# impromptuRong/hd_yolo

Hardware: AMD Instinct MI355X
Metric: tiles/sec (640x640) fwd+bwd (higher is better)
Workload: dtype bf16; 1 GPU; metayolo yolov5s 8-class nuclei, 640x640 RGB tiles, batch 64/GPU, train step = fwd + DetLoss + bwd + all-reduce + SGD(nesterov); global_batch=64, parallelism=dp1, world_size=1, backend=none, hw_queues=4

## Files before the change

### hd_yolo_amd/csrc/api.hip

```cpp
#include <stdarg.h>
#include <stdio.h>
#include <stdlib.h>
#include <string.h>

#include <atomic>

#include "common.h"
#include "hdyolo_internal.h"
#include "hdyolo.h"

int hdy_pack_weight_launch(const hdy_pack_desc& d, hipStream_t st);
int hdy_pack_batch_launch(const hdy_pack_desc* table, int n, int total_blocks, hipStream_t st);

static thread_local char g_err[512] = "";

void hdy_set_error(const char* fmt, ...) {
    va_list ap;
    va_start(ap, fmt);
    vsnprintf(g_err, sizeof(g_err), fmt, ap);
    va_end(ap);
}

namespace {
struct OptDef { const char* name; int def; bool flag; };
const OptDef g_opt_def[HDY_OPT_COUNT] = {
    {"HDY_NO_CLASS_WALK", 0, true}, {"HDY_NO_CONV3X3", 0, true}, {"HDY_C3_GRID", 0, false}, {"HDY_NO_CONV3X3S2", 0, false},
    {"HDY_NO_DGRAD_S2", 0, false}, {"HDY_TILE_INTERLEAVE", 1, false}, {"HDY_NO_BIG_TILES", 0, true}, {"HDY_NO_STEM_KERNEL", 0, true},
    {"HDY_WGRAD_BLOCKS", 512, false}, {"HDY_NO_STEM_WGRAD", 0, true}, {"HDY_NO_WGRAD3X3", 0, true}, 
    {"HDY_LOSS_GRID", 2048, false}, {"HDY_NO_DEEP", 0, true}, {"HDY_NO_WGRAD_DEEP", 0, true}, {"HDY_DEEP_BN", 0, false}, {"HDY_DEEP_DEBUG", 0, false}, {"HDY_DEEP_ALL", 1, false}, {"HDY_DEEP_MIN_TILES", 160, false}, {"HDY_DEEP_WALK", 2, false}, {"HDY_NO_BN_REDUCE4", 0, true},
    {"HDY_WGRAD_TILE", 0, false}, {"HDY_SPPF_NO_KEYS", 0, true}, {"HDY_WGRAD_DEEP_KMIN", 192, false}, {"HDY_NO_CONV3X3_C128", 0, true}, {"HDY_NO_F1X1_96", 0, true},
    {"HDY_AP_CHUNK", 0, false}, {"HDY_AP_NO_PRUNE", 0, true},
};
std::atomic<int> g_opt[HDY_OPT_COUNT];
std::once_flag g_opt_once;
void opt_init() {
    std::call_once(g_opt_once, [] {
        for (int i = 0; i < HDY_OPT_COUNT; ++i) {
            const char* v = getenv(g_opt_def[i].name);
            g_opt[i].store(v ? (g_opt_def[i].flag ? 1 : atoi(v)) : g_opt_def[i].def, std::memory_order_relaxed);
        }
    });
}
int opt_index(const char* name) {
    for (int i = 0; name && i < HDY_OPT_COUNT; ++i)
        if (!strcmp(name, g_opt_def[i].name)) return i;
    return -1;
}
thread_local char g_disp_last[64] = "";
std::mutex g_disp_mu;
char g_disp_log[32768] = "";
size_t g_disp_len = 0;
thread_local char g_disp_copy[32768] = "";
}

int hdy_opt(int id) {
    opt_init();
    return g_opt[id].load(std::memory_order_relaxed);
}

void hdy_note_dispatch(const char* what) {
    snprintf(g_disp_last, sizeof(g_disp_last), "%s", what);
    const size_t n = strlen(g_disp_last);
    std::lock_guard<std::mutex> lock(g_disp_mu);
    if (g_disp_len + n + 2 < sizeof(g_disp_log)) {
        memcpy(g_disp_log + g_disp_len, g_disp_last, n);
        g_disp_log[g_disp_len + n] = ';';
        g_disp_log[g_disp_len + n + 1] = 0;
        g_disp_len += n + 1;
    }
}

namespace {

enum { KIND_FWD = 0, KIND_DGRAD = 1, KIND_STEM = 2 };

inline int velems(int dtype) { return dtype == HDY_BF16 ? 8 : 4; }
inline int bke(int dtype) { return 8 * velems(dtype); }
inline size_t esize(int dtype) { return dtype == HDY_BF16 ? 2 : 4; }

inline size_t block_elems(int rows, int kd, int dtype) {
    const int bn = hdy_conv_bn_tile(rows);
    return (size_t)round_up(rows, bn) * round_up(kd, bke(dtype));
}

}

extern "C" {

const char* hdy_last_error(void) { return g_err; }

const char* hdy_last_dispatch(void) { return g_disp_last; }

const char* hdy_dispatch_log(void) {
    std::lock_guard<std::mutex> lock(g_disp_mu);
    memcpy(g_disp_copy, g_disp_log, g_disp_len + 1);
    return g_disp_copy;
}

void hdy_dispatch_log_reset(void) {
    std::lock_guard<std::mutex> lock(g_disp_mu);
    g_disp_log[0] = 0;
    g_disp_len = 0;
    g_disp_last[0] = 0;
}

int hdy_set_option(const char* name, int value) {
    const int i = opt_index(name);
    HDY_ARG(i >= 0, "set_option: unknown option %s", name ? name : "(null)");
    opt_init();
    return g_opt[i].exchange(value, std::memory_order_relaxed);
}

int hdy_get_option(const char* name) {
    const int i = opt_index(name);
    HDY_ARG(i >= 0, "get_option: unknown option %s", name ? name : "(null)");
    return hdy_opt(i);
}

int hdy_version(void) { return HDY_ABI_VERSION; }

int hdy_fastdiv_magic(unsigned d, unsigned* magic, int* shift) {
    HDY_ARG(d > 0 && magic && shift, "fastdiv_magic: d must be positive");
    hdy_magic(d, magic, shift);
    return HDY_OK;
}

int hdy_conv_out_dim(int in, int k, int stride, int pad) { return conv_out_dim(in, k, stride, pad); }

int hdy_conv_mtiles(long long M) { return (int)((M + 127) / 128); }

size_t hdy_conv_pack_elems(int K, int C, int R, int S, int stride, int pad, int kind, int dtype) {
    if (kind == KIND_FWD) return block_elems(K, R * S * C, dtype);
    if (kind == KIND_STEM) return block_elems(K, R * S * 4, dtype);
    if (stride == 1) return block_elems(C, R * S * K, dtype);
    size_t n = 0;
    for (int a = 0; a < 2; ++a)
        for (int b = 0; b < 2; ++b) {
            const Axis ah = class_axis(R, pad, a), aw = class_axis(S, pad, b);
            if (ah.taps && aw.taps) n += block_elems(C, ah.taps * aw.taps * K, dtype);
        }
    return n;
}

static hdy_pack_desc make_desc(const float* w_a, int K_a, const float* w_b, int K_b, void* out, int Kl, int C, int R, int S, int transpose,
                               int TH, int TW, int rbase, int rstep, int sbase, int sstep, int stem, int rows_total, int Kdp, int dtype,
                               int first_block) {
    hdy_pack_desc d = {};
    d.w_a = w_a; d.w_b = w_b; d.out = out; d.K_a = K_a; d.K_b = K_b; d.Kl = Kl; d.C = C; d.R = R; d.S = S; d.transpose = transpose;
    d.TH = TH; d.TW = TW; d.rbase = rbase; d.rstep = rstep; d.sbase = sbase; d.sstep = sstep; d.stem = stem; d.rows_total = rows_total;
    d.Kdp = Kdp; d.dtype = dtype; d.first_block = first_block;
    d.nblocks = cdiv((long long)rows_total * Kdp, 2048);
    return d;
}

int hdy_conv_pack_describe(const float* w_a, int K_a, const float* w_b, int K_b, int K, int C, int R, int S, int stride, int pad, int kind,
                           int dtype, void* out, hdy_pack_desc* descs, int first_block) {
    HDY_ARG(w_a && out && descs && K_a > 0 && K_b >= 0 && K >= K_a + K_b && C > 0 && R > 0 && S > 0, "conv_pack: bad args");
    HDY_ARG((K_b == 0) == (w_b == nullptr), "conv_pack: w_b / K_b mismatch");
    HDY_ARG(stride == 1 || stride == 2, "conv_pack: stride %d unsupported", stride);
    HDY_ARG(dtype == HDY_BF16 || dtype == HDY_F32, "conv_pack: unknown dtype %d", dtype);
    HDY_ARG(((long long)K + 256) * ((long long)R * S * ((long long)C + 256) + 64) < (1LL << 31), "conv_pack: weight too large for 32-bit packing indices");
    if (kind == KIND_FWD || kind == KIND_STEM) {
        const int stem = kind == KIND_STEM;
        HDY_ARG(!stem || (C == 3 && K_b == 0), "conv_pack: stem expects C == 3 and a single weight");
        const int kd = stem ? R * S * 4 : R * S * C;
        const int Kdp = round_up(kd, bke(dtype));
        const int rows_total = round_up(K, hdy_conv_bn_tile(K));
        descs[0] = make_desc(w_a, K_a, w_b, K_b, out, K, C, R, S, 0, R, stem ? 1 : S, 0, 1, 0, 1, stem, rows_total, Kdp, dtype, first_block);
        return 1;
    }
    HDY_ARG(kind == KIND_DGRAD, "conv_pack: unknown kind %d", kind);
    const int rows_total = round_up(C, hdy_conv_bn_tile(C));
    if (stride == 1) {
        const int Kdp = round_up(R * S * K, bke(dtype));
        descs[0] = make_desc(w_a, K_a, w_b, K_b, out, K, C, R, S, 1, R, S, R - 1, -1, S - 1, -1, 0, rows_total, Kdp, dtype, first_block);
        return 1;
    }
    size_t off = 0;
    int n = 0;
    for (int a = 0; a < 2; ++a)
        for (int b = 0; b < 2; ++b) {
            const Axis ah = class_axis(R, pad, a), aw = class_axis(S, pad, b);
            if (!ah.taps || !aw.taps) continue;
            const int Kdp = round_up(ah.taps * aw.taps * K, bke(dtype));
            descs[n] = make_desc(w_a, K_a, w_b, K_b, (char*)out + off * esize(dtype), K, C, R, S, 1, ah.taps, aw.taps, ah.rmax, -2, aw.rmax,
                                 -2, 0, rows_total, Kdp, dtype, first_block);
            first_block += descs[n].nblocks;
            off += (size_t)rows_total * Kdp;
            ++n;
        }
    return n;
}

int hdy_conv_pack(const float* w_a, int K_a, const float* w_b, int K_b, int K, int C, int R, int S, int stride, int pad, int kind,
                  int dtype, void* out, void* stream) {
    hdy_pack_desc d[4];
    const int n = hdy_conv_pack_describe(w_a, K_a, w_b, K_b, K, C, R, S, stride, pad, kind, dtype, out, d, 0);
    if (n < 0) return n;
    for (int i = 0; i < n; ++i) {
        const int rc = hdy_pack_weight_launch(d[i], (hipStream_t)stream);
        if (rc) return rc;
    }
    return HDY_OK;
}

int hdy_conv_pack_run(const hdy_pack_desc* descs_device, int ndesc, int total_blocks, void* stream) {
    HDY_ARG(descs_device && ndesc > 0 && total_blocks > 0, "conv_pack_run: bad args");
    return hdy_pack_batch_launch(descs_device, ndesc, total_blocks, (hipStream_t)stream);
}

}
```

### hd_yolo_amd/csrc/common.h

```cpp
#pragma once
#include <hip/hip_runtime.h>
#include <stdint.h>
#include <stddef.h>

#include <mutex>

#define HDY_OK 0
#define HDY_EINVAL (-1)
#define HDY_EUNSUPPORTED (-2)

enum { HDY_F32 = 0, HDY_BF16 = 1 };

void hdy_set_error(const char* fmt, ...);

enum HdyOption {
    HDY_OPT_NO_CLASS_WALK,
    HDY_OPT_NO_CONV3X3,
    HDY_OPT_C3_GRID,
    HDY_OPT_NO_CONV3X3S2,
    HDY_OPT_NO_DGRAD_S2,
    HDY_OPT_TILE_INTERLEAVE,
    HDY_OPT_NO_BIG_TILES,
    HDY_OPT_NO_STEM_KERNEL,
    HDY_OPT_WGRAD_BLOCKS,
    HDY_OPT_NO_STEM_WGRAD,
    HDY_OPT_NO_WGRAD3X3,
    HDY_OPT_LOSS_GRID,
    HDY_OPT_NO_DEEP,
    HDY_OPT_NO_WGRAD_DEEP,
    HDY_OPT_DEEP_BN,
    HDY_OPT_DEEP_DEBUG,
    HDY_OPT_DEEP_ALL,
    HDY_OPT_DEEP_MIN_TILES,
    HDY_OPT_DEEP_WALK,
    HDY_OPT_NO_BN_REDUCE4,
    HDY_OPT_WGRAD_TILE,
    HDY_OPT_SPPF_NO_KEYS,
    HDY_OPT_WGRAD_DEEP_KMIN,
    HDY_OPT_NO_CONV3X3_C128,
    HDY_OPT_NO_F1X1_96,
    HDY_OPT_AP_CHUNK,
    HDY_OPT_AP_NO_PRUNE,
    HDY_OPT_COUNT
};
int hdy_opt(int id);

void hdy_note_dispatch(const char* what);

#define HDY_ARG(cond, ...)                 \
    do {                                   \
        if (!(cond)) {                     \
            hdy_set_error(__VA_ARGS__);    \
            return HDY_EINVAL;             \
        }                                  \
    } while (0)

#define HDY_LAUNCH_CHECK(what)                                                       \
    do {                                                                             \
        hipError_t e__ = hipGetLastError();                                          \
        if (e__ != hipSuccess) {                                                     \
            hdy_set_error("%s: launch failed: %s", what, hipGetErrorString(e__));    \
            return (int)e__;                                                         \
        }                                                                            \
    } while (0)

typedef __bf16 bf16_t;
typedef int i32x4 __attribute__((ext_vector_type(4)));
typedef float f32x4 __attribute__((ext_vector_type(4)));
typedef __bf16 bf16x8 __attribute__((ext_vector_type(8)));
typedef __bf16 bf16x4 __attribute__((ext_vector_type(4)));

#if defined(__HIPCC__)
__device__ __forceinline__ float row_sum16(float v) {
#ifdef HDY_ROW_SUM_SHFL
    for (int m = 1; m < 16; m <<= 1) v += __shfl_xor(v, m);
    return v;
#endif
    v += __builtin_bit_cast(float, __builtin_amdgcn_update_dpp(0, __builtin_bit_cast(int, v), 0x128, 0xF, 0xF, true));
    v += __builtin_bit_cast(float, __builtin_amdgcn_update_dpp(0, __builtin_bit_cast(int, v), 0x124, 0xF, 0xF, true));
    v += __builtin_bit_cast(float, __builtin_amdgcn_update_dpp(0, __builtin_bit_cast(int, v), 0x122, 0xF, 0xF, true));
    v += __builtin_bit_cast(float, __builtin_amdgcn_update_dpp(0, __builtin_bit_cast(int, v), 0x121, 0xF, 0xF, true));
    return v;
}
#endif

struct PerDeviceOnce {
    std::once_flag flag[16];
    template <typename F> void run(F&& fn) {
        int dev = 0;
        (void)hipGetDevice(&dev);
        std::call_once(flag[dev & 15], fn);
    }
};

static inline int cdiv(long long a, long long b) { return (int)((a + b - 1) / b); }
static inline int round_up(int a, int b) { return (a + b - 1) / b * b; }

#ifdef __HIPCC__
union V16 {
    i32x4 i;
    f32x4 f;
    bf16x8 h;
};

__device__ __forceinline__ float silu_f(float u) { return u / (1.0f + __expf(-u)); }
__device__ __forceinline__ float sigmoid_f(float u) { return 1.0f / (1.0f + __expf(-u)); }

template <typename T> __device__ __forceinline__ float to_f32(T v);
template <> __device__ __forceinline__ float to_f32<float>(float v) { return v; }
template <> __device__ __forceinline__ float to_f32<bf16_t>(bf16_t v) { return (float)v; }
template <typename T> __device__ __forceinline__ T from_f32(float v);
template <> __device__ __forceinline__ float from_f32<float>(float v) { return v; }
template <> __device__ __forceinline__ bf16_t from_f32<bf16_t>(float v) { return (bf16_t)v; }

__device__ __forceinline__ int xcd_remap(int id, int n) {
    const int q = n >> 3, r = n & 7, x = id & 7, s = id >> 3;
    return (x < r ? x * (q + 1) : r * (q + 1) + (x - r) * q) + s;
}
__device__ __forceinline__ unsigned fdiv(unsigned n, unsigned mg, int sh) { return __umulhi(n << 1, mg) >> sh; }

__device__ __forceinline__ bool iou_gt(float ax1, float ay1, float ax2, float ay2, float aarea, float bx1, float by1, float bx2, float by2,
                                       float barea, float thr) {
    const float xx1 = ax1 > bx1 ? ax1 : bx1;
    const float yy1 = ay1 > by1 ? ay1 : by1;
    const float xx2 = ax2 < bx2 ? ax2 : bx2;
    const float yy2 = ay2 < by2 ? ay2 : by2;
    float w = __fsub_rn(xx2, xx1);
    float h = __fsub_rn(yy2, yy1);
    w = w < 0.f ? 0.f : w;
    h = h < 0.f ? 0.f : h;
    const float inter = __fmul_rn(w, h);
    const float ovr = __fdiv_rn(inter, __fsub_rn(__fadd_rn(aarea, barea), inter));
    return ovr > thr;
}

__device__ __forceinline__ unsigned desc_key(float s) {
    unsigned u = s == 0.0f ? 0u : __float_as_uint(s);
    u = (u & 0x80000000u) ? ~u : (u | 0x80000000u);
    return ~u;
}

__device__ __forceinline__ void glds16(const void* g, unsigned char* lds_wave_base) {
    __builtin_amdgcn_global_load_lds((const void __attribute__((address_space(1)))*)g,
                                     (void __attribute__((address_space(3)))*)lds_wave_base, 16, 0, 0);
}

__device__ __forceinline__ void lds_dma16(__amdgpu_buffer_rsrc_t r, unsigned voff, unsigned soff, unsigned char* lds_wave_base) {
    __builtin_amdgcn_raw_ptr_buffer_load_lds(r, (void __attribute__((address_space(3)))*)lds_wave_base, 16, (int)voff, (int)soff, 0, 0);
}

__device__ __forceinline__ void lds_dma16(__amdgpu_buffer_rsrc_t r, unsigned voff, unsigned soff, unsigned lds_byte) {
    __builtin_amdgcn_raw_ptr_buffer_load_lds(r, (void __attribute__((address_space(3)))*)(uintptr_t)lds_byte, 16, (int)voff, (int)soff, 0, 0);
}

__device__ __forceinline__ int fsw(int row) { return ((row >> 1) & 1) | (((row >> 3) & 1) << 1); }
__device__ __forceinline__ int fsw3(int row) { return (row & 6) ^ (((row >> 3) & 1) * 5); }

__device__ __forceinline__ float fast_sigmoid(float u) { return __builtin_amdgcn_rcpf(1.0f + __expf(-u)); }
__device__ __forceinline__ float dsilu_f(float u) {
    const float s = fast_sigmoid(u);
    return s * (1.0f + u * (1.0f - s));
}

template <typename T> __device__ __forceinline__ void unpack(const i32x4& v, float* f);
template <> __device__ __forceinline__ void unpack<float>(const i32x4& v, float* f) {
    V16 u; u.i = v;
#pragma unroll
    for (int i = 0; i < 4; ++i) f[i] = u.f[i];
}
template <> __device__ __forceinline__ void unpack<bf16_t>(const i32x4& v, float* f) {
    V16 u; u.i = v;
#pragma unroll
    for (int i = 0; i < 8; ++i) f[i] = (float)u.h[i];
}
template <typename T> __device__ __forceinline__ i32x4 pack(const float* f);
template <> __device__ __forceinline__ i32x4 pack<float>(const float* f) {
    V16 u;
#pragma unroll
    for (int i = 0; i < 4; ++i) u.f[i] = f[i];
    return u.i;
}
template <> __device__ __forceinline__ i32x4 pack<bf16_t>(const float* f) {
    V16 u;
#pragma unroll
    for (int i = 0; i < 8; ++i) u.h[i] = (bf16_t)f[i];
    return u.i;
}

#define VEC_OK(ptr, ld, VE) ((((uintptr_t)(ptr)) & 15) == 0 && (ld) % (VE) == 0)

#define S2_LDSR(dst, addr)                                                                             \
    do {                                                                                               \
        if constexpr (HAND) asm volatile("ds_read_b128 %0, %1" : "=v"(dst) : "v"(addr) : "memory");    \
        else dst = *(const i32x4*)(smem + ((addr) - lds0));                                            \
    } while (0)
#define S2_LGKM(n)                                                                                                       \
    do {                                                                                                                 \
        if constexpr (HAND) { asm volatile("s_waitcnt lgkmcnt(%0)" ::"n"(n) : "memory"); __builtin_amdgcn_sched_barrier(0); } \
    } while (0)
#define S2_BARRIER(lg)                                                                                                   \
    do {                                                                                                                 \
        if constexpr (HAND) { if (lg) asm volatile("s_waitcnt lgkmcnt(0)" ::: "memory"); __builtin_amdgcn_s_barrier(); asm volatile("" ::: "memory"); } \
        else __syncthreads();                                                                                            \
    } while (0)
#endif
```

### hd_yolo_amd/csrc/conv_dgrad_s2.hip

```cpp
#include <stdlib.h>

#include "common.h"
#include "hdyolo_internal.h"

__device__ uint4 g_hdy_zero16_d2[4];

namespace {

constexpr int TW = 16, PW = TW + 1;
constexpr int CB = 128, CPP = 8;

template <int NP, int NCG, int TH> struct Geo {
    static constexpr int NWP = TH / 4;
    static constexpr int NTHR = 64 * NCG * NWP;
    static constexpr int PPIX = (TH + 1) * PW;
    static constexpr int PLANE_B = PPIX * CB;
    static constexpr int PATCH_B = NP * PLANE_B;
    static constexpr int PPR = 4 / NCG;
    static constexpr int RPH = 32 / PPR;
    static constexpr int SROWS = 2 * TH * RPH;
    static constexpr int STAGE_B = SROWS * 128;
    static constexpr int SMEM_B = 2 * PATCH_B + STAGE_B;
    static constexpr int NPASS = (PPIX * CPP + NTHR - 1) / NTHR;
    static constexpr int RPP = NTHR / 8;
    static constexpr int SPASS = SROWS / RPP;
    static constexpr int HSTEP = RPP / RPH;
    static_assert(SPASS == 8 && RPP % RPH == 0 && PPIX <= 153, "geometry");
};

template <int NP, int NCG, int TH, int ABL = 0>
__global__ __launch_bounds__(64 * NCG * (TH / 4), 2) void dgrad3x3s2_kernel(const ConvArgs p) {
    using G = Geo<NP, NCG, TH>;
    constexpr int NTHR = G::NTHR, PATCH_B = G::PATCH_B, PLANE_B = G::PLANE_B, PPIX = G::PPIX, NPASS = G::NPASS, PPR = G::PPR, KD = 64 * NP;
    constexpr bool HAND = NP == 2;
    extern __shared__ __attribute__((aligned(16))) unsigned char smem[];
    unsigned char* sP = smem;
    unsigned char* sS = smem + 2 * PATCH_B;

    const unsigned lds0 = (unsigned)(uintptr_t)(const __attribute__((address_space(3))) unsigned char*)smem;
    const int tid = threadIdx.x, lane = tid & 63, wave = tid >> 6;
    const int fr = lane & 15, fq = lane >> 4;
    const int wc = wave % NCG, wp = wave / NCG;
    const int tiles_w = p.Wo / TW, tiles_h = p.Ho / TH, per_img = tiles_w * tiles_h;
    const int tiles = p.N * per_img;
    const int wg = xcd_remap(blockIdx.x, gridDim.x);

    const bf16_t* __restrict__ x = (const bf16_t*)p.x;
    const bf16_t* __restrict__ w = (const bf16_t*)p.w;
    const unsigned char* zero = (const unsigned char*)g_hdy_zero16_d2;

    V16 bw[9][2 * NP];
    {
        constexpr int cls_of[9] = {0, 1, 1, 2, 2, 3, 3, 3, 3}, tap_of[9] = {0, 0, 1, 0, 1, 0, 1, 2, 3};
#pragma unroll
        for (int i = 0; i < 9; ++i) {
            const bf16_t* base = w + p.c_w[cls_of[i]] + (size_t)(wc * 16 + fr) * (p.c_nkb[cls_of[i]] * 64) + tap_of[i] * KD;
#pragma unroll
            for (int kk = 0; kk < 2 * NP; ++kk) bw[i][kk].i = *(const i32x4*)(base + (kk * 4 + fq) * 8);
        }
    }

    auto issue_patch = [&](int t, int buf) {
        int tv = tid;
        if constexpr (HAND) asm volatile("" : "+v"(tv));
        const int lc = tv & 7, wv = tv >> 6;
        const int n = t / per_img, rem = t - n * per_img;
        const int th = rem / tiles_w, tw = rem - th * tiles_w;
        const int i0 = th * TH, j0 = tw * TW;
        const bf16_t* org = x + (((long long)n * p.Hin + i0) * p.Win + j0) * p.ldx;
        unsigned char* dst = sP + buf * PATCH_B;
#pragma unroll
        for (int pl = 0; pl < NP; ++pl)
#pragma unroll
            for (int i = 0; i < NPASS; ++i) {
                if ((wave * 64 + NTHR * i) / CPP >= PPIX) break;
                const int pix = (tv + NTHR * i) / CPP;
                if (pix >= PPIX) continue;
                const int py = (pix * 3856) >> 16, px = pix - py * PW;
                const int lcp = lc ^ (((px >> 1) & 3) << 1);
                const void* src = (i0 + py < p.Hin && j0 + px < p.Win) ? (const void*)(org + ((long long)py * p.Win + px) * p.ldx + pl * 64 + lcp * 8) : (const void*)zero;
                glds16(src, dst + pl * PLANE_B + (wv * 64 + NTHR * i) * 16);
            }
    };

    int aoff[2][2];
#pragma unroll
    for (int s = 0; s < 2; ++s)
#pragma unroll
        for (int ks = 0; ks < 2; ++ks) {
            const int px = fr + s;
            aoff[s][ks] = px * CB + (((ks * 4 + fq) ^ (((px >> 1) & 3) << 1)) << 4);
        }

    const int st_ch = tid & 7, st_rr = tid >> 3;
    const int st_key = PPR == 2 ? (st_rr & 15) : ((st_rr >> 1) & 15);
    const int st_lds = st_rr * 128 + ((st_ch ^ (st_key >> 1)) << 4);
    const int st_hr0 = st_rr / G::RPH;
    const long long st_pix = PPR == 2 ? (long long)(2 * (st_rr & 15) + (st_ch >> 2)) * p.ldy + (st_ch & 3) * 8 : (long long)(st_rr & 31) * p.ldy + st_ch * 8;

    auto compute = [&](int t, int cur) {
        f32x4 acc[4][4];
#pragma unroll
        for (int c = 0; c < 4; ++c)
#pragma unroll
            for (int a = 0; a < 4; ++a) acc[c][a] = f32x4{0.f, 0.f, 0.f, 0.f};
#pragma unroll
        for (int pl = 0; pl < NP; ++pl) {
            const unsigned pb = lds0 + cur * PATCH_B + pl * PLANE_B + wp * 4 * PW * CB;
            V16 f[2][2];
            S2_LDSR(f[0][0].i, pb + aoff[0][0]);
            S2_LDSR(f[0][1].i, pb + aoff[1][0]);
#pragma unroll
            for (int g = 0; g < 10; ++g) {
                const int q = g >> 1, ks = pl * 2 + (g & 1);
                if (g + 1 < 10) {
                    S2_LDSR(f[(g + 1) & 1][0].i, pb + ((g + 1) >> 1) * PW * CB + aoff[0][(g + 1) & 1]);
                    S2_LDSR(f[(g + 1) & 1][1].i, pb + ((g + 1) >> 1) * PW * CB + aoff[1][(g + 1) & 1]);
                    S2_LGKM(2);
                } else {
                    S2_LGKM(0);
                }
                const bf16x8 f0 = f[g & 1][0].h, f1 = f[g & 1][1].h;
                if (ABL & 4) continue;
                if (q < 4) {
                    acc[0][q] = __builtin_amdgcn_mfma_f32_16x16x32_bf16(bw[0][ks].h, f0, acc[0][q], 0, 0, 0);
                    acc[1][q] = __builtin_amdgcn_mfma_f32_16x16x32_bf16(bw[1][ks].h, f0, acc[1][q], 0, 0, 0);
                    acc[2][q] = __builtin_amdgcn_mfma_f32_16x16x32_bf16(bw[3][ks].h, f0, acc[2][q], 0, 0, 0);
                    acc[3][q] = __builtin_amdgcn_mfma_f32_16x16x32_bf16(bw[5][ks].h, f0, acc[3][q], 0, 0, 0);
                    acc[1][q] = __builtin_amdgcn_mfma_f32_16x16x32_bf16(bw[2][ks].h, f1, acc[1][q], 0, 0, 0);
                    acc[3][q] = __builtin_amdgcn_mfma_f32_16x16x32_bf16(bw[6][ks].h, f1, acc[3][q], 0, 0, 0);
                }
                if (q >= 1) {
                    acc[2][q - 1] = __builtin_amdgcn_mfma_f32_16x16x32_bf16(bw[4][ks].h, f0, acc[2][q - 1], 0, 0, 0);
                    acc[3][q - 1] = __builtin_amdgcn_mfma_f32_16x16x32_bf16(bw[7][ks].h, f0, acc[3][q - 1], 0, 0, 0);
                    acc[3][q - 1] = __builtin_amdgcn_mfma_f32_16x16x32_bf16(bw[8][ks].h, f1, acc[3][q - 1], 0, 0, 0);
                }
            }
        }
#pragma unroll
        for (int c = 0; c < 4; ++c)
#pragma unroll
            for (int a = 0; a < 4; ++a) {
                const int ca = c >> 1, cb = c & 1;
                const int hr = 2 * (wp * 4 + a) + ca;
                const int R = PPR == 2 ? hr * 16 + fr : hr * 32 + 2 * fr + cb;
                const int slot = PPR == 2 ? cb * 8 + wc * 4 + fq : wc * 4 + fq;
                bf16x4 o = {(bf16_t)acc[c][a][0], (bf16_t)acc[c][a][1], (bf16_t)acc[c][a][2], (bf16_t)acc[c][a][3]};
                *(bf16x4*)(sS + R * 128 + ((slot ^ (fr & 15)) << 3)) = o;
            }
        S2_BARRIER(true);
        {
            const int n = t / per_img, rem = t - n * per_img;
            const int th = rem / tiles_w, tw = rem - th * tiles_w;
            bf16_t* yb = (bf16_t*)p.y + (((long long)n * p.Hout + 2 * th * TH + st_hr0) * p.Wout + 2 * tw * TW) * p.ldy + st_pix;
            const long long st_step = (long long)G::HSTEP * p.Wout * p.ldy;
            V16 v[8];
#pragma unroll
            for (int j = 0; j < 8; ++j) S2_LDSR(v[j].i, lds0 + 2 * PATCH_B + st_lds + j * G::RPP * 128);
            S2_LGKM(0);
            if (p.accumulate) {
                V16 u[8];
#pragma unroll
                for (int j = 0; j < 8; ++j) u[j].i = *(const i32x4*)(yb + j * st_step);
#pragma unroll
                for (int j = 0; j < 8; ++j) {
                    if (st_key & 1) v[j].i = i32x4{v[j].i[2], v[j].i[3], v[j].i[0], v[j].i[1]};
#pragma unroll
                    for (int e = 0; e < 8; ++e) v[j].h[e] = (bf16_t)((float)v[j].h[e] + (float)u[j].h[e]);
                }
            } else {
#pragma unroll
                for (int j = 0; j < 8; ++j)
                    if (st_key & 1) v[j].i = i32x4{v[j].i[2], v[j].i[3], v[j].i[0], v[j].i[1]};
            }
#pragma unroll
            for (int j = 0; j < 8; ++j) {
                if (ABL & 8) break;
                *(i32x4*)(yb + j * st_step) = v[j].i;
            }
        }
        asm volatile("s_waitcnt vmcnt(8)" ::: "memory");
        S2_BARRIER(false);
    };

    if (wg >= tiles) return;
    if ((ABL & 16) && blockIdx.x >= gridDim.x / 2) __builtin_amdgcn_s_sleep(90);
    issue_patch(wg, 0);
    asm volatile("s_waitcnt vmcnt(0)" ::: "memory");
    __syncthreads();
    int cur = 0;
    for (int t = wg; t < tiles; t += (int)gridDim.x, cur ^= 1) {
        if (t + (int)gridDim.x < tiles && !(ABL & 1)) issue_patch(t + (int)gridDim.x, cur ^ 1);
        compute(t, cur);
    }
}

}

template <int NP, int NCG, int TH>
static int dgrad_s2_launch(const ConvArgs& a, int grid, hipStream_t st) {
    using G = Geo<NP, NCG, TH>;
    static PerDeviceOnce attr_once;
    attr_once.run([&] {
        (void)hipFuncSetAttribute((const void*)dgrad3x3s2_kernel<NP, NCG, TH>, hipFuncAttributeMaxDynamicSharedMemorySize, G::SMEM_B);
    });
#ifdef HDY_PROBE_BUILD
    const int abl = hdy_opt(HDY_OPT_DEEP_DEBUG);
    if constexpr (NP == 2) if (abl) {
#define ABL_CASE(v) if (abl == v) { (void)hipFuncSetAttribute((const void*)dgrad3x3s2_kernel<NP, NCG, TH, v>, hipFuncAttributeMaxDynamicSharedMemorySize, G::SMEM_B); hipLaunchKernelGGL((dgrad3x3s2_kernel<NP, NCG, TH, v>), dim3(grid), dim3(G::NTHR), G::SMEM_B, st, a); return (int)hipGetLastError(); }
        ABL_CASE(1) ABL_CASE(4) ABL_CASE(8) ABL_CASE(12) ABL_CASE(9) ABL_CASE(5) ABL_CASE(16)
#undef ABL_CASE
    }
#endif
    hipLaunchKernelGGL((dgrad3x3s2_kernel<NP, NCG, TH>), dim3(grid), dim3(G::NTHR), G::SMEM_B, st, a);
    return hdy_launch_status("dgrad3x3s2");
}

bool hdy_dgrad3x3s2_plan(const ConvShape& s, ConvPlan* p) {
    const int disabled = hdy_opt(HDY_OPT_NO_DGRAD_S2);
    if (disabled == 1 || s.dtype != HDY_BF16 || s.ncls != 4 || s.stats || s.R != 3 || s.S != 3 || s.stride != 2 || s.pad != 1) return false;
    const int planes = (s.C == 64 && s.K == 32) ? 1 : ((s.C == 128 && s.K == 64 && disabled != 2) ? 2 : 0);
    const int th = planes == 1 ? 8 : 4;
    if (!planes || s.Ho % th || s.Wo % TW) return false;
    const int tiles = s.N * (s.Ho / th) * (s.Wo / TW);
    *p = ConvPlan{CONV_DGRAD_S2, planes, tiles < 512 ? tiles : 512, 0, 0, 0};
    return true;
}

int hdy_dgrad3x3s2_launch(const ConvArgs& a, const ConvPlan& p, int out_f32, hipStream_t st) {
    if (out_f32 || a.res || a.scale || a.shift || a.act != 0) return HDY_CONV_DECLINE;
    const bool aligned = rows_aligned(a, true) && a.c_w[0] % 8 == 0 && a.c_w[1] % 8 == 0 && a.c_w[2] % 8 == 0 && a.c_w[3] % 8 == 0;
    if (const int rc = hdy_conv_take(a, p, aligned, "dgrad3x3s2")) return rc;
    hdy_note_dispatch(p.variant == 1 ? "dgrad3x3s2_k64c32" : "dgrad3x3s2_k128c64");
    return p.variant == 1 ? dgrad_s2_launch<1, 2, 8>(a, p.grid, st) : dgrad_s2_launch<2, 4, 4>(a, p.grid, st);
}
```

Baseline: 5489 tiles/s.

## Add wide stride-2 3x3 dgrad kernel for deeper channel counts

Adds a new specialized stride-2 3x3 data-gradient kernel for K of 128/256 and C from 128 to 1024. It uses 20-wide tiles over two sub-images, a 3-slot LDS ring of filter and patch chunks with async global-to-LDS loads, and 16x16x32 bf16 MFMAs. It is enabled by default when the deep-walk mode is 2 and there are enough pixels. These layers previously fell back to the generic dgrad path; the new path is meant to reuse patches across taps and to overlap loads with compute. The cost is a large new hand-scheduled kernel, one workgroup per CU, and a cap of 256 workgroups on the grid.

```diff
diff --git a/hd_yolo_amd/csrc/api.hip b/hd_yolo_amd/csrc/api.hip
--- a/hd_yolo_amd/csrc/api.hip
+++ b/hd_yolo_amd/csrc/api.hip
@@ -29,7 +29,7 @@
     {"HDY_WGRAD_BLOCKS", 512, false}, {"HDY_NO_STEM_WGRAD", 0, true}, {"HDY_NO_WGRAD3X3", 0, true}, 
     {"HDY_LOSS_GRID", 2048, false}, {"HDY_NO_DEEP", 0, true}, {"HDY_NO_WGRAD_DEEP", 0, true}, {"HDY_DEEP_BN", 0, false}, {"HDY_DEEP_DEBUG", 0, false}, {"HDY_DEEP_ALL", 1, false}, {"HDY_DEEP_MIN_TILES", 160, false}, {"HDY_DEEP_WALK", 2, false}, {"HDY_NO_BN_REDUCE4", 0, true},
     {"HDY_WGRAD_TILE", 0, false}, {"HDY_SPPF_NO_KEYS", 0, true}, {"HDY_WGRAD_DEEP_KMIN", 192, false}, {"HDY_NO_CONV3X3_C128", 0, true}, {"HDY_NO_F1X1_96", 0, true},
-    {"HDY_AP_CHUNK", 0, false}, {"HDY_AP_NO_PRUNE", 0, true},
+    {"HDY_AP_CHUNK", 0, false}, {"HDY_AP_NO_PRUNE", 0, true}, {"HDY_DGRAD_S2_WIDE", 1, false},
 };
 std::atomic<int> g_opt[HDY_OPT_COUNT];
 std::once_flag g_opt_once;
diff --git a/hd_yolo_amd/csrc/common.h b/hd_yolo_amd/csrc/common.h
--- a/hd_yolo_amd/csrc/common.h
+++ b/hd_yolo_amd/csrc/common.h
@@ -41,6 +41,7 @@
     HDY_OPT_NO_F1X1_96,
     HDY_OPT_AP_CHUNK,
     HDY_OPT_AP_NO_PRUNE,
+    HDY_OPT_DGRAD_S2_WIDE,
     HDY_OPT_COUNT
 };
 int hdy_opt(int id);
diff --git a/hd_yolo_amd/csrc/conv_dgrad_s2.hip b/hd_yolo_amd/csrc/conv_dgrad_s2.hip
--- a/hd_yolo_amd/csrc/conv_dgrad_s2.hip
+++ b/hd_yolo_amd/csrc/conv_dgrad_s2.hip
@@ -4,6 +4,8 @@
 #include "hdyolo_internal.h"
 
 __device__ uint4 g_hdy_zero16_d2[4];
+constexpr int WIDE_MAX_KD = 1024;
+__device__ uint4 g_hdy_zero_wide[WIDE_MAX_KD * 2 / 16 + 1];
 
 namespace {
 
@@ -195,6 +197,245 @@
     }
 }
 
+namespace wide {
+constexpr int TH = 4, TW = 20, PW = TW + 1, NSUB = 2, NPOS = NSUB * TH * TW, SPIX = (TH + 1) * PW, PPIX = NSUB * SPIX;
+constexpr int CBK = 64;
+constexpr int NTHR = 512;
+constexpr int ROW_B = 64;
+constexpr int FILT_B = 9 * CBK * ROW_B;
+constexpr int PATCH_B = 224 * ROW_B;
+constexpr int UNIT_B = FILT_B + PATCH_B;
+constexpr int NPIECE = UNIT_B / 1024;
+constexpr int NDMA = 7;
+constexpr int RING = 3;
+constexpr int SMEM_B = RING * UNIT_B + 1024;
+constexpr int STAGE_ROWS = 2 * NPOS;
+constexpr int NST = STAGE_ROWS * 8 / NTHR;
+static_assert(NDMA * 8 >= NPIECE && PPIX * ROW_B <= PATCH_B && STAGE_ROWS * 128 <= UNIT_B && NST * NTHR == STAGE_ROWS * 8 && SMEM_B <= 160 * 1024, "geometry");
+
+__device__ __forceinline__ int swz(int row) { return (4 - ((row >> 2) & 3)) & 3; }
+
+#define WIDE_MFMA(a, b, c, x, y, z) ((ABL & 4) ? (c) : __builtin_amdgcn_mfma_f32_16x16x32_bf16(a, b, c, x, y, z))
+#define WIDE_LDSR(dst, addr, off) asm volatile("ds_read_b128 %0, %1 offset:%2" : "=v"(dst) : "v"(addr), "n"(off) : "memory")
+
+template <int ABL = 0>
+__global__ __launch_bounds__(NTHR, 1) void dgrad3x3s2_wide_kernel(const ConvArgs p) {
+    constexpr bool HAND = true;
+    extern __shared__ __attribute__((aligned(16))) unsigned char smem[];
+    const unsigned lds0 = (unsigned)(uintptr_t)(const __attribute__((address_space(3))) unsigned char*)smem;
+    const int tid = threadIdx.x, lane = tid & 63, wave = __builtin_amdgcn_readfirstlane(tid >> 6);
+    const int fr = lane & 15, fq = lane >> 4;
+    const int wc = wave & 3, wp = wave >> 2;
+    const int tiles_w = p.Wo / TW, qpi = p.Ho / TH;
+    const int tiles = (p.N * qpi / NSUB) * tiles_w, items = tiles * (p.K / CBK);
+    const int KD = p.C, upi = 2 * (KD / 64);
+    const int G = (int)gridDim.x, wg = xcd_remap(blockIdx.x, G);
+    if (wg >= items) return;
+    const int nunits = ((items - wg + G - 1) / G) * upi;
+
+    const bf16_t* __restrict__ x = (const bf16_t*)p.x;
+    const bf16_t* __restrict__ w = (const bf16_t*)p.w;
+    const bf16_t* zero = (const bf16_t*)g_hdy_zero_wide;
+
+    unsigned ld_off[NDMA];
+    int ld_flag[NDMA];
+#pragma unroll
+    for (int j = 0; j < NDMA; ++j) {
+        const int piece = wave + 8 * j;
+        if (piece < 36) {
+            const int i = piece >> 2, cls = i == 0 ? 0 : (i < 3 ? 1 : (i < 5 ? 2 : 3)), tap = i - (cls == 0 ? 0 : (cls == 1 ? 1 : (cls == 2 ? 3 : 5)));
+            const int nkb = cls == 0 ? p.c_nkb[0] : (cls == 1 ? p.c_nkb[1] : (cls == 2 ? p.c_nkb[2] : p.c_nkb[3]));
+            const int row = (piece & 3) * 16 + (lane >> 2);
+            ld_off[j] = (unsigned)(row * (nkb * 64) + tap * KD + (((lane & 3) ^ swz(row)) << 3));
+            ld_flag[j] = 0;
+        } else {
+            const int q = (piece - 36) * 64 + lane, pix = q >> 2, sub = pix >= SPIX ? 1 : 0, sp = pix - sub * SPIX;
+            const int py = sp / PW, px = sp - py * PW;
+            ld_off[j] = (unsigned)((py * p.Win + px) * p.ldx + (((q & 3) ^ swz(pix)) << 3));
+            ld_flag[j] = (piece >= NPIECE || pix >= PPIX ? 1 : 0) | (py == TH ? 2 : 0) | (px == TW ? 4 : 0) | (sub ? 8 : 0);
+        }
+    }
+
+    const bf16_t* src[NDMA];
+    auto item_sources = [&](int m) {
+        const int it = wg + m * G, cb = it / tiles, t = it - cb * tiles;
+        const int qp = t / tiles_w, tw = t - qp * tiles_w, j0 = tw * TW;
+        const int n0 = (NSUB * qp) / qpi, i0 = ((NSUB * qp) - n0 * qpi) * TH;
+        const int n1 = (NSUB * qp + 1) / qpi, i1 = ((NSUB * qp + 1) - n1 * qpi) * TH;
+        const bool last_r0 = i0 + TH >= p.Hin, last_r1 = i1 + TH >= p.Hin, last_c = j0 + TW >= p.Win;
+        const bf16_t* xo0 = x + (((long long)n0 * p.Hin + i0) * p.Win + j0) * p.ldx;
+        const bf16_t* xo1 = x + (((long long)n1 * p.Hin + i1) * p.Win + j0) * p.ldx;
+#pragma unroll
+        for (int j = 0; j < NDMA; ++j) {
+            const int piece = wave + 8 * j;
+            if (piece < 36) {
+                const int i = piece >> 2, cls = i == 0 ? 0 : (i < 3 ? 1 : (i < 5 ? 2 : 3));
+                const long long cw = cls == 0 ? p.c_w[0] : (cls == 1 ? p.c_w[1] : (cls == 2 ? p.c_w[2] : p.c_w[3]));
+                const int nkb = cls == 0 ? p.c_nkb[0] : (cls == 1 ? p.c_nkb[1] : (cls == 2 ? p.c_nkb[2] : p.c_nkb[3]));
+                src[j] = w + (cw + (long long)cb * CBK * (nkb * 64)) + ld_off[j];
+            } else {
+                const int f = ld_flag[j];
+                const bool out = (f & 1) || ((f & 2) && ((f & 8) ? last_r1 : last_r0)) || ((f & 4) && last_c);
+                src[j] = out ? zero : ((f & 8) ? xo1 : xo0) + ld_off[j];
+            }
+        }
+    };
+    int iu_r = 0, iu_m = 0;
+    auto issue = [&](int slot) {
+        if (iu_r == 0) item_sources(iu_m);
+        unsigned char* dst = smem + slot * UNIT_B;
+#pragma unroll
+        for (int j = 0; j < NDMA; ++j) {
+            const int piece = wave + 8 * j;
+            if (!(ABL & 1) || iu_m + iu_r < 2) glds16(src[j], piece < NPIECE ? dst + piece * 1024 : smem + RING * UNIT_B);
+            src[j] += 32;
+        }
+        if (++iu_r == upi) { iu_r = 0; ++iu_m; }
+    };
+
+    const unsigned f_off = (unsigned)((wc * 16 + fr) * ROW_B + ((fq ^ swz(fr)) << 4));
+    unsigned d_off[5][4];
+#pragma unroll
+    for (int f = 0; f < 5; ++f) {
+        const int lp = f * 16 + fr, row = lp / TW, col = lp - row * TW;
+#pragma unroll
+        for (int s = 0; s < 4; ++s) {
+            const int pp = wp * SPIX + (row + (s >> 1)) * PW + col + (s & 1);
+            d_off[f][s] = (unsigned)(FILT_B + pp * ROW_B + ((fq ^ swz(pp)) << 4));
+        }
+    }
+
+    f32x4 acc[4][5];
+#pragma unroll
+    for (int c = 0; c < 4; ++c)
+#pragma unroll
+        for (int f = 0; f < 5; ++f) acc[c][f] = f32x4{0.f, 0.f, 0.f, 0.f};
+
+    if constexpr ((ABL & 16) != 0) {
+        for (int i = 0; i < (int)(blockIdx.x >> 3 & 3); ++i) __builtin_amdgcn_s_sleep(42);
+    }
+    issue(0);
+    issue(1);
+    int skip = 0;
+    for (int u = 0, r = 0, m = 0, slot = 0; u < nunits; ++u, slot = slot == RING - 1 ? 0 : slot + 1) {
+        if (skip > 0) --skip;
+        else if (u + 1 < nunits) asm volatile("s_waitcnt vmcnt(7)" ::: "memory");
+        else asm volatile("s_waitcnt vmcnt(0)" ::: "memory");
+        S2_BARRIER(false);
+        if (u + 2 < nunits) issue(slot == 0 ? RING - 1 : slot - 1);
+
+        const unsigned ub = lds0 + slot * UNIT_B;
+        if (!(ABL & 2) || u == 0) {
+            V16 bw[9], d[2][5];
+            const unsigned fb = ub + f_off;
+            WIDE_LDSR(bw[0].i, fb, 0 * 4096); WIDE_LDSR(bw[1].i, fb, 1 * 4096); WIDE_LDSR(bw[3].i, fb, 3 * 4096); WIDE_LDSR(bw[5].i, fb, 5 * 4096);
+#pragma unroll
+            for (int f = 0; f < 5; ++f) WIDE_LDSR(d[0][f].i, ub + d_off[f][0], 0);
+            WIDE_LDSR(bw[2].i, fb, 2 * 4096); WIDE_LDSR(bw[6].i, fb, 6 * 4096);
+#pragma unroll
+            for (int f = 0; f < 5; ++f) WIDE_LDSR(d[1][f].i, ub + d_off[f][1], 0);
+            S2_LGKM(7);
+#pragma unroll
+            for (int f = 0; f < 5; ++f) acc[0][f] = WIDE_MFMA(bw[0].h, d[0][f].h, acc[0][f], 0, 0, 0);
+#pragma unroll
+            for (int f = 0; f < 5; ++f) acc[1][f] = WIDE_MFMA(bw[1].h, d[0][f].h, acc[1][f], 0, 0, 0);
+#pragma unroll
+            for (int f = 0; f < 5; ++f) acc[2][f] = WIDE_MFMA(bw[3].h, d[0][f].h, acc[2][f], 0, 0, 0);
+#pragma unroll
+            for (int f = 0; f < 5; ++f) acc[3][f] = WIDE_MFMA(bw[5].h, d[0][f].h, acc[3][f], 0, 0, 0);
+            WIDE_LDSR(bw[4].i, fb, 4 * 4096); WIDE_LDSR(bw[7].i, fb, 7 * 4096);
+#pragma unroll
+            for (int f = 0; f < 5; ++f) WIDE_LDSR(d[0][f].i, ub + d_off[f][2], 0);
+            S2_LGKM(7);
+#pragma unroll
+            for (int f = 0; f < 5; ++f) acc[1][f] = WIDE_MFMA(bw[2].h, d[1][f].h, acc[1][f], 0, 0, 0);
+#pragma unroll
+            for (int f = 0; f < 5; ++f) acc[3][f] = WIDE_MFMA(bw[6].h, d[1][f].h, acc[3][f], 0, 0, 0);
+            WIDE_LDSR(bw[8].i, fb, 8 * 4096);
+#pragma unroll
+            for (int f = 0; f < 5; ++f) WIDE_LDSR(d[1][f].i, ub + d_off[f][3], 0);
+            S2_LGKM(6);
+#pragma unroll
+            for (int f = 0; f < 5; ++f) acc[2][f] = WIDE_MFMA(bw[4].h, d[0][f].h, acc[2][f], 0, 0, 0);
+#pragma unroll
+            for (int f = 0; f < 5; ++f) acc[3][f] = WIDE_MFMA(bw[7].h, d[0][f].h, acc[3][f], 0, 0, 0);
+            S2_LGKM(0);
+#pragma unroll
+            for (int f = 0; f < 5; ++f) acc[3][f] = WIDE_MFMA(bw[8].h, d[1][f].h, acc[3][f], 0, 0, 0);
+        }
+        if (++r < upi) continue;
+        if (ABL & 8) { r = 0; ++m; continue; }
+
+        {
+            const int it = wg + m * G, cb = it / tiles, t = it - cb * tiles;
+            const int qp = t / tiles_w, tw = t - qp * tiles_w;
+            const int n0 = (NSUB * qp) / qpi, i0 = ((NSUB * qp) - n0 * qpi) * TH, n1 = (NSUB * qp + 1) / qpi, i1 = ((NSUB * qp + 1) - n1 * qpi) * TH;
+            bf16_t* yt = (bf16_t*)p.y + (long long)(2 * tw * TW) * p.ldy + cb * CBK + (tid & 7) * 8;
+            bf16_t* yb0 = yt + ((long long)n0 * p.Hout + 2 * i0) * p.Wout * p.ldy;
+            bf16_t* yb1 = yt + ((long long)n1 * p.Hout + 2 * i1) * p.Wout * p.ldy;
+            unsigned char* sS = smem + slot * UNIT_B;
+            asm volatile("s_waitcnt vmcnt(0)" ::: "memory");
+            skip = 2;
+#pragma unroll
+            for (int ca = 0; ca < 2; ++ca) {
+                S2_BARRIER(false);
+#pragma unroll
+                for (int cbit = 0; cbit < 2; ++cbit)
+#pragma unroll
+                    for (int f = 0; f < 5; ++f) {
+                        const int pos = wp * 80 + f * 16 + fr, R = pos * 2 + cbit;
+                        const f32x4 a = acc[ca * 2 + cbit][f];
+                        bf16x4 o = {(bf16_t)a[0], (bf16_t)a[1], (bf16_t)a[2], (bf16_t)a[3]};
+                        *(bf16x4*)(sS + R * 128 + (((wc * 4 + fq) ^ (pos & 15)) << 3)) = o;
+                        acc[ca * 2 + cbit][f] = f32x4{0.f, 0.f, 0.f, 0.f};
+                    }
+                S2_BARRIER(true);
+                V16 v[NST];
+                bf16_t* yo[NST];
+#pragma unroll
+                for (int j = 0; j < NST; ++j) {
+                    const int R = (tid >> 3) + 64 * j, key = (R >> 1) & 15;
+                    const int sub = R >= 160 ? 1 : 0, Rs = R - sub * 160, hr = Rs / 40, px = Rs - hr * 40;
+                    yo[j] = (sub ? yb1 : yb0) + ((long long)(2 * hr + ca) * p.Wout + px) * p.ldy;
+                    WIDE_LDSR(v[j].i, ub + (unsigned)(R * 128 + (((tid & 7) ^ (key >> 1)) << 4)), 0);
+                }
+                S2_LGKM(0);
+#pragma unroll
+                for (int j = 0; j < NST; ++j)
+                    if ((((tid >> 3) + 64 * j) >> 1) & 1) v[j].i = i32x4{v[j].i[2], v[j].i[3], v[j].i[0], v[j].i[1]};
+                if (p.accumulate) {
+                    V16 o[NST];
+#pragma unroll
+                    for (int j = 0; j < NST; ++j) o[j].i = *(const i32x4*)yo[j];
+#pragma unroll
+                    for (int j = 0; j < NST; ++j)
+#pragma unroll
+                        for (int e = 0; e < 8; ++e) v[j].h[e] = (bf16_t)((float)v[j].h[e] + (float)o[j].h[e]);
+                }
+#pragma unroll
+                for (int j = 0; j < NST; ++j) *(i32x4*)yo[j] = v[j].i;
+            }
+            r = 0; ++m;
+        }
+    }
+}
+#undef WIDE_LDSR
+#undef WIDE_MFMA
+}
+
+}
+
+static int dgrad_s2_wide_launch(const ConvArgs& a, int grid, hipStream_t st) {
+    static PerDeviceOnce attr_once;
+    attr_once.run([&] { (void)hipFuncSetAttribute((const void*)wide::dgrad3x3s2_wide_kernel<0>, hipFuncAttributeMaxDynamicSharedMemorySize, wide::SMEM_B); });
+#ifdef HDY_PROBE_BUILD
+    const int abl = hdy_opt(HDY_OPT_DEEP_DEBUG);
+#define ABL_CASE(v) if (abl == v) { (void)hipFuncSetAttribute((const void*)wide::dgrad3x3s2_wide_kernel<v>, hipFuncAttributeMaxDynamicSharedMemorySize, wide::SMEM_B); hipLaunchKernelGGL(wide::dgrad3x3s2_wide_kernel<v>, dim3(grid), dim3(wide::NTHR), wide::SMEM_B, st, a); return (int)hipGetLastError(); }
+    ABL_CASE(1) ABL_CASE(2) ABL_CASE(4) ABL_CASE(8) ABL_CASE(6) ABL_CASE(7) ABL_CASE(9) ABL_CASE(14) ABL_CASE(15) ABL_CASE(16)
+#undef ABL_CASE
+#endif
+    hipLaunchKernelGGL(wide::dgrad3x3s2_wide_kernel<0>, dim3(grid), dim3(wide::NTHR), wide::SMEM_B, st, a);
+    return hdy_launch_status("dgrad3x3s2_wide");
 }
 
 template <int NP, int NCG, int TH>
@@ -216,9 +457,21 @@
     return hdy_launch_status("dgrad3x3s2");
 }
 
+static bool dgrad_s2_wide_plan(const ConvShape& s, ConvPlan* p) {
+    const int opt = hdy_opt(HDY_OPT_DGRAD_S2_WIDE);
+    if (opt == 0 || hdy_opt(HDY_OPT_DEEP_WALK) != 2) return false;
+    if (s.C % 64 || s.C < 128 || s.C > WIDE_MAX_KD || (s.K != 128 && s.K != 256) || s.Ho % wide::TH || s.Wo % wide::TW || (s.N * (s.Ho / wide::TH)) % wide::NSUB) return false;
+    if (opt < 2 && conv_pixels(s) < 8192) return false;
+    const long long items = (long long)(s.N * (s.Ho / wide::TH) / wide::NSUB) * (s.Wo / wide::TW) * (s.K / wide::CBK);
+    const int cap = opt > 2 ? opt : 256;
+    *p = ConvPlan{CONV_DGRAD_S2, 3, (int)(items < cap ? items : cap), 0, 0, 0};
+    return true;
+}
+
 bool hdy_dgrad3x3s2_plan(const ConvShape& s, ConvPlan* p) {
     const int disabled = hdy_opt(HDY_OPT_NO_DGRAD_S2);
     if (disabled == 1 || s.dtype != HDY_BF16 || s.ncls != 4 || s.stats || s.R != 3 || s.S != 3 || s.stride != 2 || s.pad != 1) return false;
+    if (dgrad_s2_wide_plan(s, p)) return true;
     const int planes = (s.C == 64 && s.K == 32) ? 1 : ((s.C == 128 && s.K == 64 && disabled != 2) ? 2 : 0);
     const int th = planes == 1 ? 8 : 4;
     if (!planes || s.Ho % th || s.Wo % TW) return false;
@@ -231,6 +484,10 @@
     if (out_f32 || a.res || a.scale || a.shift || a.act != 0) return HDY_CONV_DECLINE;
     const bool aligned = rows_aligned(a, true) && a.c_w[0] % 8 == 0 && a.c_w[1] % 8 == 0 && a.c_w[2] % 8 == 0 && a.c_w[3] % 8 == 0;
     if (const int rc = hdy_conv_take(a, p, aligned, "dgrad3x3s2")) return rc;
+    if (p.variant == 3) {
+        hdy_note_dispatch("dgrad3x3s2_wide");
+        return dgrad_s2_wide_launch(a, p.grid, st);
+    }
     hdy_note_dispatch(p.variant == 1 ? "dgrad3x3s2_k64c32" : "dgrad3x3s2_k128c64");
     return p.variant == 1 ? dgrad_s2_launch<1, 2, 8>(a, p.grid, st) : dgrad_s2_launch<2, 4, 4>(a, p.grid, st);
 }
```

New measurement: 5510 tiles/s (median of 6 runs). No clear change (+0.4%).
